# omerbt/Splice

Hardware: AMD Instinct MI355X
Metric: opt_steps_per_sec (higher is better)
Workload: dtype bf16

## Files before the change

include/splice_hip.h:

```cpp
#ifndef SPLICE_HIP_H
#define SPLICE_HIP_H
#include <stddef.h>
#include <stdint.h>

#ifdef __cplusplus
extern "C" {
#endif

typedef uint16_t splice_bf16;
typedef void* splice_stream_t;

#define SPLICE_OK 0
#define SPLICE_ERR_ARG -1
#define SPLICE_ERR_HIP -2
#define SPLICE_ERR_STATE -3
#define SPLICE_ERR_NOMEM -4

int splice_version(void);
int splice_dev_switches(void);
const char* splice_last_error(void);

typedef struct splice_gemm_epilogue {
    const float* bias;
    const float* resid;
// ... 280 lines not shown
int splice_rows_finish(int mode, const float* slabs, int n_slabs, size_t slab_stride, int rows, int N, const float* bias, const float* resid, size_t rs,
                       float* out_f32, size_t os, splice_bf16* out_bf, splice_bf16* pre_bf, const splice_bf16* aux, size_t ps, int pre_lo,
                       splice_stream_t stream);

typedef struct splice_gen_conv_args {
    const float* in;
    const float* w;
    const float* bias;
    float* out;
    size_t in_nstride, in_cstride, out_nstride, out_cstride, w_jstride, w_cstride, p_nstride;
    int N, Cin, Hi, Wi, Cout, Ho, Wo, ks, stride, pad;
    int reflect, act, transposed, accumulate;
    float* ws;
    size_t ws_floats;
    int p_group, defer_reduce;
} splice_gen_conv_args;
#define SPLICE_GEN_CONV_FORM_INTS 5
int splice_gen_conv(const splice_gen_conv_args* args, int* form_out, splice_stream_t stream);
int splice_gen_conv_pair(const splice_gen_conv_args* a, const splice_gen_conv_args* b, int* forms_out, splice_stream_t stream);
int splice_gen_conv_reflect_dgrad(const splice_gen_conv_args* args, float* pad_scratch, size_t scratch_floats, splice_stream_t stream);

typedef struct splice_gen_wgrad_args {
    const float* x;
    const float* dy;
    float* ws;
    size_t ws_floats;
    size_t x_nstride, x_cstride, dy_nstride, dy_cstride;
    int N, Cin, Hi, Wi, Cout, Ho, Wo, ks, stride, pad, reflect;
} splice_gen_wgrad_args;
#define SPLICE_GEN_WGRAD_FORM_INTS 6
size_t splice_gen_conv_wgrad_ws_floats(int N, int Cin, int Cout, int ks, int Ho, int Wo);
int splice_gen_conv_wgrad(const splice_gen_wgrad_args* args, float* dw, int accumulate, int n_img, size_t p_nstride, int* form_out,
                          splice_stream_t stream);
int splice_gen_wgrad_reduce(const float* partials, int n, int chunks, float* dw, int accumulate, int n_img, size_t p_nstride, splice_stream_t stream);

typedef struct splice_gen_bn_args {
    float* y;
    float* out;
    size_t y_nstride, out_nstride;
    int N, C, HW, batch;
    const float* gamma;
    const float* beta;
    float eps, slope;
    size_t p_nstride;
    float* part;
    size_t part_floats;
    float* mean;
    float* rstd;
    const float* up_src;
    float* up_d_src;
    size_t up_src_ns, up_d_src_ns;
    int up_c0, up_h, up_w, up_Ho, up_Wo;
    const float* slabs;
    const float* bias;
    int ksplit;
    const float* da;
    float* dy;
    size_t da_nstride, dy_nstride;
    float* dgamma;
    float* dbeta;
    int accumulate;
    const float* da_slabs;
    int da_ksplit, da_accumulate;
    float* pre_y;
    size_t pre_y_ns;
    const float* pre_slabs;
// ... 31 lines not shown
```

splice_amd/_lib.py:

```python
import ctypes as C
import os

_HERE = os.path.dirname(os.path.abspath(__file__))
LIB_PATH = os.path.join(_HERE, "libsplice_hip.so")

_lib = None


class GemmEpilogue(C.Structure):
    _fields_ = [
        ("bias", C.c_void_p), ("resid", C.c_void_p), ("ldr", C.c_int), ("resid_mod", C.c_int),
        ("out_f32", C.c_void_p), ("ldo", C.c_int),
        ("out_bf", C.c_void_p), ("ldbf", C.c_int),
        ("out_bf_t", C.c_void_p), ("ldt", C.c_int),
        ("out_pre", C.c_void_p), ("ldp", C.c_int), ("pre_row_lo", C.c_int),
        ("aux", C.c_void_p), ("ldaux", C.c_int),
        ("out_f32_cols", C.c_void_p), ("ld_cols", C.c_int), ("col_lo", C.c_int), ("col_hi", C.c_int),
        ("alpha", C.c_float), ("ksplit", C.c_int), ("slab_stride", C.c_longlong),
        ("rd_other", C.c_void_p), ("ld_rd", C.c_int), ("rd_rows", C.c_int), ("rowdot", C.c_void_p),
        ("row_scale", C.c_void_p), ("col_scale", C.c_void_p),
        ("out_f8", C.c_void_p), ("ld8", C.c_int),
        ("out_f8_t", C.c_void_p), ("ldt8", C.c_int),
    ]

# ... 78 lines not shown
    "splice_gemm_nt_bf16": ([_u, _vp, _i, _vp, _i, _i, _i, _i, C.POINTER(GemmEpilogue), _vp], _i),
    "splice_gemm_nt_fp8": ([_u, _vp, _i, _vp, _i, _i, _i, _i, C.POINTER(GemmEpilogue), _vp], _i),
    "splice_quantize_rows_fp8": ([_vp, _i, _vp, _i, _vp, _i, _i, _vp], _i),
    "splice_gemm_splitk_slabs": ([_i, _i], _i),
    "splice_gemm_force_tile": ([_i], _i),
    "splice_attention_variant": ([_i], _i),
    "splice_attention_qfold": ([_i], _i),
    "splice_attention_bwd_variant": ([_i], _i),
    "splice_layernorm_fwd": ([_vp, _vp, _vp, _vp, _vp, _vp, _i, _i, _f, _vp], _i),
    "splice_layernorm_bwd": ([_vp, _vp, _vp, _vp, _vp, _vp, _vp, _vp, _i, _i, _vp], _i),
    "splice_attention_fwd": ([_vp, _vp, _i, _i, _i, _i, _i, _i, _f, _vp, _vp, _vp], _i),
    "splice_attention_fwd_fp8": ([_vp, _vp, _i, _i, _i, _i, _i, _i, _f, _vp, _vp, _vp], _i),
    "splice_attention_bwd": ([_vp, _vp, _i, _i, _i, _i, _i, _i, _f, _vp, _vp, _vp, _vp, _vp, _vp, _vp], _i),
    "splice_attention_probs": ([_vp, _i, _i, _i, _i, _i, _f, _vp, _vp, _vp], _i),
    "splice_augment_structure": ([_vp, _vp, _vp, _i, _i, _i, _i, C.POINTER(C.c_int), C.POINTER(C.c_float), _f, _vp], _i),
    "splice_keys_selfsim_ws_bytes": ([_i, _i], _sz),
    "splice_keys_selfsim_fwd": ([_vp, _i, _i, _i, _f, _vp, _vp, _vp], _i),
    "splice_keys_selfsim_bwd": ([_vp, _vp, _i, _i, _f, _vp, _i, _i, _vp, _vp], _i),
    "splice_mse": ([_vp, _i, _vp, _i, _i, _i, _f, _vp, _vp, _i, _vp], _i),
    "splice_selfsim_loss_pairs_ws_bytes": ([_i, _i, _i], _sz),
    "splice_selfsim_loss_pairs": ([_vp, _vp, _i, _sz, _vp, _i, _sz, _i, _i, _i, _f, _vp, _i, _f, _vp, _sz, _vp, _i, _sz, _vp, _vp], _i),
    "splice_mse_pairs": ([_vp, _i, _sz, _vp, _i, _sz, _i, _i, _f, _f, _vp, _sz, _vp, _i, _sz, _i, _vp, _vp], _i),
    "splice_total_loss_pairs": ([_vp, _sz, _i, _f, _f, _f, _f, _f, _vp, _i, _i, _i, _i, _i, _vp, _i, _i, _vp], _i),
    "splice_attn_cls_fwd": ([_vp, _vp, _i, _i, _i, _i, _i, _i, _f, _vp, _vp, _vp], _i),
    "splice_attn_cls_bwd": ([_vp, _vp, _i, _i, _i, _i, _i, _i, _f, _vp, _vp, _i, _sz, _vp, _vp], _i),
    "splice_ln_rows_fwd": ([_vp, _sz, _vp, _vp, _vp, _sz, _vp, _vp, _sz, _i, _i, _f, _vp, _i, _sz, _vp, _vp, _sz, _vp], _i),
    "splice_ln_rows_bwd": ([_vp, _sz, _vp, _sz, _vp, _vp, _vp, _sz, _vp, _vp, _i, _i, _i, _sz, _vp], _i),
    "splice_rows_finish": ([_i, _vp, _i, _sz, _i, _i, _vp, _vp, _sz, _vp, _sz, _vp, _vp, _vp, _sz, _i, _vp], _i),
    "splice_gen_conv": ([C.POINTER(GenConvArgs), C.POINTER(_i), _vp], _i),
    "splice_gen_conv_pair": ([C.POINTER(GenConvArgs), C.POINTER(GenConvArgs), C.POINTER(_i), _vp], _i),
    "splice_gen_conv_reflect_dgrad": ([C.POINTER(GenConvArgs), _vp, _sz, _vp], _i),
    "splice_gen_conv_wgrad_ws_floats": ([_i, _i, _i, _i, _i, _i], _sz),
    "splice_gen_conv_wgrad": ([C.POINTER(GenWgradArgs), _vp, _i, _i, _sz, C.POINTER(_i), _vp], _i),
    "splice_gen_wgrad_reduce": ([_vp, _i, _i, _vp, _i, _i, _sz, _vp], _i),
    "splice_gen_bn_small_instance": ([_i], _i),
    "splice_gen_bn_form": ([_i, _i, _sz, _i, C.POINTER(_i)], _i),
    "splice_gen_bn_part_floats": ([_i, _i], _sz),
    "splice_gen_bn_fwd": ([C.POINTER(GenBnArgs), _vp], _i),
    "splice_gen_bn_bwd": ([C.POINTER(GenBnArgs), _vp], _i),
    "splice_gen_upsample2x_fwd": ([_vp, _sz, _vp, _sz, _i, _i, _i, _i, _i, _i, _vp], _i),
    "splice_gen_upsample2x_bwd": ([_vp, _sz, _vp, _sz, _i, _i, _i, _i, _i, _i, _vp], _i),
    "splice_gen_sigmoid_bias_part_floats": ([_i, _i], _sz),
    "splice_gen_sigmoid_bwd_bias": ([_vp, _vp, _vp, _i, _i, _i, _vp, _sz, _sz, _i, C.POINTER(_i), _vp], _i),
    "splice_patchify": ([_vp, _vp, _i, _i, _i, _i, _i, _i, _vp], _i),
    "splice_unpatchify": ([_vp, _vp, _i, _i, _i, _i, _i, _i, _vp], _i),
    "splice_cast_f32_bf16": ([_vp, _vp, _sz, _vp], _i),
    "splice_cast_bf16_f32": ([_vp, _vp, _sz, _vp], _i),
    "splice_transpose_f32_bf16": ([_vp, _vp, _i, _i, _i, _vp], _i),
    "splice_resize_bilinear_fwd": ([_vp, _vp, _i, _i, _i, _i, _i, _vp], _i),
    "splice_resize_bilinear_bwd": ([_vp, _vp, _i, _i, _i, _i, _i, _vp], _i),
    "splice_vit_create": ([_i, _i, _i, _i, C.POINTER(_vp)], _i),
    "splice_vit_destroy": ([_vp], None),
    "splice_vit_set_param": ([_vp, C.c_char_p, _vp, C.c_longlong, _vp], _i),
    "splice_vit_params_complete": ([_vp], _i),
    "splice_vit_enable_fp8": ([_vp, _vp], _i),
    "splice_vit_ctx_create": ([_vp, _i, _i, _i, _vp, _i, _vp, C.POINTER(_vp)], _i),
    "splice_vit_ctx_destroy": ([_vp], None),
    "splice_vit_ctx_info": ([_vp, C.POINTER(_i), C.POINTER(_i), C.POINTER(_i)], _i),
    "splice_vit_ctx_set_top_cls_only": ([_vp, _i], _i),
    "splice_vit_ctx_set_fp8": ([_vp, _i], _i),
    "splice_vit_forward": ([_vp, _vp, _i, _vp], _i),
    "splice_vit_forward_ex": ([_vp, _vp, _i, _i, _vp], _i),
    "splice_vit_forward_passes": ([_vp, _vp, _i, _i, _i, _i, _vp], _i),
    "splice_vit_get_tensor": ([_vp, _i, _i, C.POINTER(_vp)], _i),
    "splice_vit_qscale": ([_vp], C.c_float),
    "splice_vit_read_tensor": ([_vp, _i, _i, _vp, _sz, _vp], _i),
# ... 103 lines not shown
```

splice_amd/csrc/capi.hip:

```cpp
#include <stdarg.h>
#include <stdio.h>

#include "gen_kernels.h"
#include "kernels.h"

static thread_local char g_err[512] = "";

void splice_set_error(const char* fmt, ...) {
    va_list ap;
    va_start(ap, fmt);
    vsnprintf(g_err, sizeof(g_err), fmt, ap);
    va_end(ap);
}

static int finish(int rc, const char* what) {
    if (rc != SPLICE_OK) {
        splice_set_error("%s: invalid argument", what);
        return rc;
    }
    const hipError_t e = hipGetLastError();
    if (e != hipSuccess) {
        splice_set_error("%s: HIP error %d (%s)", what, (int)e, hipGetErrorString(e));
        return SPLICE_ERR_HIP;
    }
// ... 252 lines not shown
    return (size_t)wgrad_chunks(N, Ho, Wo, &ppc, &cpi) * Cout * Cin * ks * ks;
}
int splice_gen_conv_wgrad(const splice_gen_wgrad_args* args, float* dw, int accumulate, int n_img, size_t p_nstride, int* form_out, splice_stream_t stream) {
    const char* who = "splice_gen_conv_wgrad";
    if (!gen_wgrad_args_ok(args) || !dw || !args->ws) return finish(SPLICE_ERR_ARG, who);
    const size_t n = (size_t)args->Cout * args->Cin * args->ks * args->ks;
    if (n > 0x7fffffffULL || args->ws_floats < splice_gen_conv_wgrad_ws_floats(args->N, args->Cin, args->Cout, args->ks, args->Ho, args->Wo))
        return finish(SPLICE_ERR_ARG, who);
    if (p_nstride ? (n_img != args->N || p_nstride < n) : n_img != 1) return finish(SPLICE_ERR_ARG, who);
    WgradArgs a = {};
    a.x = args->x; a.dy = args->dy; a.ws = args->ws;
    a.x_nstride = args->x_nstride; a.x_cstride = args->x_cstride; a.dy_nstride = args->dy_nstride; a.dy_cstride = args->dy_cstride;
    a.N = args->N; a.Cin = args->Cin; a.Hi = args->Hi; a.Wi = args->Wi; a.Cout = args->Cout; a.Ho = args->Ho; a.Wo = args->Wo;
    a.ks = args->ks; a.stride = args->stride; a.pad = args->pad; a.reflect = args->reflect;
    WgradBatchPair pair = {};
    int chunks = 0;
    int rc = conv_wgrad_add(&pair, a, &chunks);
    if (rc != SPLICE_OK) return finish(rc, who);
    WgradReduceAll r = {};
    r.count = 1; r.n[0] = (int)n; r.chunks[0] = chunks; r.ws_off[0] = 0; r.dw_off[0] = 0;
    if (form_out) {
        const WgradBatch& b = pair.tile.count ? pair.tile : pair.big.count ? pair.big : pair.small;
        form_out[0] = pair.tile.count ? 2 : pair.big.count ? 1 : 0;
        form_out[1] = b.d[0].variant;
        form_out[2] = b.d[0].pix_per_chunk;
        form_out[3] = chunks;
        form_out[4] = !((reinterpret_cast<size_t>(args->ws) | reinterpret_cast<size_t>(dw)) & 15) && p_nstride % 4 == 0 && n % 4 == 0;
        form_out[5] = b.total_wgs;
    }
    rc = conv_wgrad_batched_launch(pair, ST(stream));
    if (rc != SPLICE_OK) return finish(rc, who);
    return finish(wgrad_reduce_all_launch(r, args->ws, dw, accumulate, ST(stream), n_img, p_nstride), who);
}

int splice_gen_wgrad_reduce(const float* partials, int n, int chunks, float* dw, int accumulate, int n_img, size_t p_nstride, splice_stream_t stream) {
    const char* who = "splice_gen_wgrad_reduce";
    if (!partials || !dw || n < 1 || chunks < 0 || n_img < 1 || n_img > 65535 || (long long)n * (chunks > 0 ? chunks : 1) > 0x7fffffffLL) return finish(SPLICE_ERR_ARG, who);
    if (p_nstride ? (chunks % n_img || p_nstride < (size_t)n) : n_img != 1) return finish(SPLICE_ERR_ARG, who);
    WgradReduceAll r = {};
    r.count = 1; r.n[0] = n; r.chunks[0] = chunks; r.ws_off[0] = 0; r.dw_off[0] = 0;
    return finish(wgrad_reduce_all_launch(r, partials, dw, accumulate, ST(stream), n_img, p_nstride), who);
}

int splice_gen_bn_small_instance(int mask) { return finish(bn_small_force_instance(mask), "splice_gen_bn_small_instance"); }
int splice_gen_bn_form(int HW, int N, size_t p_nstride, int batch, int* out) {
    if (HW < 1 || N < 1 || batch < 0 || !out) return finish(SPLICE_ERR_ARG, "splice_gen_bn_form");
    const BnForm f = bn_form(HW, N, p_nstride, batch);
    out[0] = (int)f.kind; out[1] = f.hosts_pre; out[2] = f.fwd_takes_slabs; out[3] = f.bwd_takes_slabs;
    out[4] = f.fwd_fuses_upsample; out[5] = f.bwd_fuses_upsample; out[6] = f.sign_from_y;
    return SPLICE_OK;
}
size_t splice_gen_bn_part_floats(int N, int C) { return N < 1 || C < 1 ? 0 : (size_t)bn_part_floats(N, C); }
static bool gen_bn_fill(const splice_gen_bn_args* g, bool bwd, BnArgs* a, BnUpsample* up, BnPre* pre, BnSlabs* sl) {
    if (!g || !g->y || !g->out || !g->gamma || !g->mean || !g->rstd) return false;
    if (g->N < 1 || g->C < 1 || g->HW < 1 || g->N > 65535 || g->C > 65535 || g->batch < 0 || g->batch > 8) return false;
    if (g->batch && (g->N % g->batch || (g->N != g->batch && !g->p_nstride))) return false;
    if (g->N > 1 && (g->y_nstride < (size_t)g->C * g->HW || g->out_nstride < (size_t)g->C * g->HW)) return false;
    const BnForm f = bn_form(g->HW, g->N, g->p_nstride, g->batch);
    const bool two_stage = f.kind == BnForm::TWO_STAGE || f.kind == BnForm::TWO_STAGE_VEC;
    if (two_stage && (!g->part || g->part_floats < (size_t)bn_part_floats(g->N, g->C))) return false;
    if (!bwd && !g->beta) return false;
    if (bwd && ((f.sign_from_y && !g->beta) || !g->da || !g->dy || !g->dgamma || !g->dbeta)) return false;
    if (bwd && g->N > 1 && (g->da_nstride < (size_t)g->C * g->HW || g->dy_nstride < (size_t)g->C * g->HW)) return false;
    a->y = g->y; a->y_nstride = g->y_nstride; a->out = g->out; a->out_nstride = g->out_nstride;
    a->N = g->N; a->C = g->C; a->HW = g->HW; a->gamma = g->gamma; a->beta = g->beta; a->eps = g->eps; a->slope = g->slope;
    a->p_nstride = g->p_nstride; a->batch = g->batch; a->part = g->part; a->mean = g->mean; a->rstd = g->rstd;
// ... 95 lines not shown
```

splice_amd/csrc/gen_wgrad.hip:

```cpp
#include "gen_device.h"
#include <cstdlib>

constexpr int WG_PC = 64;
constexpr int WG_LD = WG_PC + 2;
constexpr int WG_XS_FLOATS = 3 * 16 * WG_LD;
constexpr int WG_DS_FLOATS = 8 * 16 * WG_LD;
template <int KS, int NI, bool ROWS = false>
__device__ __forceinline__ void conv_wgrad_body(const WgradArgs& a, int chunk, int ktile_in, float* Xs, float* Ds) {
    constexpr int T = ROWS ? KS : KS * KS;
    constexpr int CK = (ROWS || KS == 3) ? 4 : 16;
    constexpr int KT = CK * T;
    const int ktile = ROWS ? ktile_in / KS : ktile_in;
    const int krow = ROWS ? ktile_in % KS : 0;
    constexpr int NJ = (KT + 15) / 16;
    constexpr int PC = WG_PC;
    constexpr int LD = WG_LD;
    constexpr int NQ = (NI * NJ + 3) / 4;
    constexpr int NA = KT / 4;
    constexpr int ND = NI * 16 * PC / 256;
    const int tid = threadIdx.x, lane = tid & 63, wave = tid >> 6;
    const int c0 = ktile * CK;
    const int HWo = a.Ho * a.Wo;
    const int chunks_per_img = a.chunks_per_img;
    const int img = chunk / chunks_per_img, ch_in_img = chunk % chunks_per_img;
    const float* x = a.x + (size_t)img * a.x_nstride + (size_t)c0 * a.x_cstride;
    const float* dy = a.dy + (size_t)img * a.dy_nstride;
    f32x4 acc[NQ];
#pragma unroll
    for (int q = 0; q < NQ; ++q) acc[q] = f32x4{0.f, 0.f, 0.f, 0.f};
    for (int e = tid; e < (NJ * 16 - KT) * LD; e += 256) Xs[KT * LD + e] = 0.f;
    const int pl = tid & 63;
    const int p_begin = ch_in_img * a.pix_per_chunk;
    const int p_end = min(p_begin + a.pix_per_chunk, HWo);
    const int wave_g = (KS == 3 && NI == 8) ? __builtin_amdgcn_readfirstlane(wave) : wave;
    int g_coff[NA], g_dy[NA], g_dx[NA];
    unsigned g_cok = 0;
#pragma unroll
    for (int i = 0; i < NA; ++i) {
        const int k = wave_g + 4 * i;
        const int cl = k / T, tap = k % T;
        g_coff[i] = (int)(cl * a.x_cstride);
        g_dy[i] = (ROWS ? krow : tap / KS) - a.pad;
        g_dx[i] = (ROWS ? tap : tap % KS) - a.pad;
        if (c0 + cl < a.Cin) g_cok |= 1u << i;
    }
    float xv[NA], dv[ND];
    const __amdgpu_buffer_rsrc_t rx = __builtin_amdgcn_make_buffer_rsrc(const_cast<float*>(x), 0, 0x7FFFFFFF, 0x00020000);
    const __amdgpu_buffer_rsrc_t rdy = __builtin_amdgcn_make_buffer_rsrc(const_cast<float*>(dy), 0, 0x7FFFFFFF, 0x00020000);
    int d_vo[ND];
#pragma unroll
    for (int t = 0; t < ND; ++t) {
        const int e = tid + 256 * t;
        const int n = e / PC, q = e % PC;
        d_vo[t] = n < a.Cout ? (int)((n * a.dy_cstride + q) * 4) : (int)0x80000000;
    }
    auto fetch = [&](int pb) {
        const int p = pb + pl;
        const bool pvalid = p < p_end;
        const int oy = pvalid ? p / a.Wo : 0, ox = pvalid ? p % a.Wo : 0;
        const int by = oy * a.stride, bx = ox * a.stride;
#pragma unroll
        for (int i = 0; i < NA; ++i) {
            int sy = by + g_dy[i], sx = bx + g_dx[i];
            if (a.reflect) {
                sy = sy < 0 ? -sy : (sy >= a.Hi ? 2 * (a.Hi - 1) - sy : sy);
                sx = sx < 0 ? -sx : (sx >= a.Wi ? 2 * (a.Wi - 1) - sx : sx);
            }
            const bool ok = pvalid && ((g_cok >> i) & 1u) && (unsigned)sy < (unsigned)a.Hi && (unsigned)sx < (unsigned)a.Wi;
            const int vo = ok ? (g_coff[i] + sy * a.Wi + sx) * 4 : (int)0x80000000;
            xv[i] = __builtin_bit_cast(float, __builtin_amdgcn_raw_buffer_load_b32(rx, vo, 0, 0));
        }
        if (pb + PC <= p_end) {
            const int so = __builtin_amdgcn_readfirstlane(pb * 4);
#pragma unroll
            for (int t = 0; t < ND; ++t) dv[t] = __builtin_bit_cast(float, __builtin_amdgcn_raw_buffer_load_b32(rdy, d_vo[t], so, 0));
        } else {
#pragma unroll
            for (int t = 0; t < ND; ++t) {
                const int e = tid + 256 * t;
                const int n = e / PC, q = e % PC;
                const int pp = pb + q;
                dv[t] = (n < a.Cout && pp < p_end) ? dy[(size_t)n * a.dy_cstride + pp] : 0.f;
            }
        }
    };
    fetch(p_begin);
    constexpr int WB = 4, NB = PC / 4 / WB;
    [[maybe_unused]] int lds_rd = (lane & 15) * LD + (lane >> 4);
    for (int pb = p_begin; pb < p_end; pb += PC) {
        if constexpr (NI < 4) asm volatile("" : "+v"(lds_rd));
        __syncthreads();
#pragma unroll
        for (int i = 0; i < NA; ++i) Xs[(wave + 4 * i) * LD + pl] = xv[i];
#pragma unroll
        for (int t = 0; t < ND; ++t) {
            const int e = tid + 256 * t;
            Ds[(e / PC) * LD + (e % PC)] = dv[t];
        }
        __syncthreads();
        if (pb + PC < p_end) fetch(pb + PC);
#pragma unroll
        for (int q = 0; q < NQ; ++q) {
            const int pair = wave + 4 * q;
            if (pair < NI * NJ) {
                const int fi = pair / NJ, fj = pair % NJ;
                if constexpr (NI >= 4) {
#pragma unroll
                    for (int s4 = 0; s4 < PC / 4; ++s4) {
                        const float av = Ds[(fi * 16 + (lane & 15)) * LD + s4 * 4 + (lane >> 4)];
                        const float bv = Xs[(fj * 16 + (lane & 15)) * LD + s4 * 4 + (lane >> 4)];
                        acc[q] = mfma4(av, bv, acc[q]);
                    }
                } else {
                    const int d_rd = lds_rd + fi * 16 * LD, x_rd = lds_rd + fj * 16 * LD;
                    float af[2][WB], bf[2][WB];
#pragma unroll
                    for (int t = 0; t < WB; ++t) { af[0][t] = Ds[d_rd + t * 4]; bf[0][t] = Xs[x_rd + t * 4]; }
#pragma unroll
                    for (int b = 0; b < NB; ++b) {
                        if (b + 1 < NB) {
#pragma unroll
                            for (int t = 0; t < WB; ++t) { af[(b + 1) & 1][t] = Ds[d_rd + ((b + 1) * WB + t) * 4]; bf[(b + 1) & 1][t] = Xs[x_rd + ((b + 1) * WB + t) * 4]; }
                        }
                        __builtin_amdgcn_sched_barrier(0);
#pragma unroll
                        for (int t = 0; t < WB; ++t) acc[q] = mfma4(af[b & 1][t], bf[b & 1][t], acc[q]);
                        __builtin_amdgcn_sched_barrier(0);
                    }
                }
            }
        }
    }
    constexpr int TT = KS * KS;
    float* ws = a.ws + (size_t)chunk * a.Cout * a.Cin * TT;
#pragma unroll
    for (int q = 0; q < NQ; ++q) {
        const int pair = wave + 4 * q;
        if (pair < NI * NJ) {
            const int fi = pair / NJ, fj = pair % NJ;
            const int k = fj * 16 + (lane & 15);
            const int cl = k / T, tap = k % T;
            if (k < KT && c0 + cl < a.Cin) {
#pragma unroll
                for (int r = 0; r < 4; ++r) {
                    const int n = fi * 16 + (lane >> 4) * 4 + r;
                    if (n < a.Cout) ws[((size_t)n * a.Cin + c0 + cl) * TT + (ROWS ? krow * KS + tap : tap)] = acc[q][r];
                }
            }
        }
    }
}

__device__ __forceinline__ void wgrad_loaded(float& x) { asm volatile("" : "+v"(x) : : "memory"); }
template <class Load>
__device__ __forceinline__ float wgrad_chunk_sum(int chunks, Load&& ld) {
    float s0 = 0.f, s1 = 0.f, s2 = 0.f, s3 = 0.f;
    int c = 0;
#pragma unroll 1
    for (; c + 31 < chunks; c += 32) {
        float v[32];
#pragma unroll
        for (int u = 0; u < 32; ++u) v[u] = ld(c + u);
#pragma unroll
        for (int u = 0; u < 32; ++u) wgrad_loaded(v[u]);
#pragma unroll
        for (int u = 0; u < 32; u += 4) { s0 += v[u]; s1 += v[u + 1]; s2 += v[u + 2]; s3 += v[u + 3]; }
    }
    for (; c + 15 < chunks; c += 16) {
        float v[16];
#pragma unroll
        for (int u = 0; u < 16; ++u) v[u] = ld(c + u);
#pragma unroll
        for (int u = 0; u < 16; u += 4) { s0 += v[u]; s1 += v[u + 1]; s2 += v[u + 2]; s3 += v[u + 3]; }
    }
    for (; c + 3 < chunks; c += 4) {
        s0 += ld(c);
        s1 += ld(c + 1);
        s2 += ld(c + 2);
        s3 += ld(c + 3);
    }
    for (; c < chunks; ++c) s0 += ld(c);
    return (s0 + s1) + (s2 + s3);
}
// ... 61 lines not shown
            a1.x += v1.x; a1.y += v1.y; a1.z += v1.z; a1.w += v1.w;
            a2.x += v2.x; a2.y += v2.y; a2.z += v2.z; a2.w += v2.w;
            a3.x += v3.x; a3.y += v3.y; a3.z += v3.z; a3.w += v3.w;
        }
        for (; c < chunks; ++c) {
            const float4 v0 = *reinterpret_cast<const float4*>(p + (size_t)c * n);
            a0.x += v0.x; a0.y += v0.y; a0.z += v0.z; a0.w += v0.w;
        }
        s.x = (a0.x + a1.x) + (a2.x + a3.x); s.y = (a0.y + a1.y) + (a2.y + a3.y);
        s.z = (a0.z + a1.z) + (a2.z + a3.z); s.w = (a0.w + a1.w) + (a2.w + a3.w);
        float4* q4 = reinterpret_cast<float4*>(q);
        if (accumulate) { const float4 o = *q4; s.x = o.x + s.x; s.y = o.y + s.y; s.z = o.z + s.z; s.w = o.w + s.w; }
        *q4 = s;
        return;
    }
    const float s = wgrad_chunk_sum(chunks, [&](int c) { return p[(size_t)c * n]; });
    *q = accumulate ? *q + s : s;
}

int wgrad_chunks(int N, int Ho, int Wo, int* pix_per_chunk, int* chunks_per_img) {
    const int HWo = Ho * Wo;
    int ppc = 512;
    if (HWo <= 1024) ppc = 256;
    if (HWo <= 256) ppc = 64;
    if (HWo > 128 * 512) ppc = (cdiv(HWo, 128) + 63) / 64 * 64;
    *pix_per_chunk = ppc;
    *chunks_per_img = cdiv(HWo, ppc);
    return N * *chunks_per_img;
}

template <bool BIG>
__global__ __launch_bounds__(256, 2) void conv_wgrad_batched_kernel(WgradBatch b) {
    __shared__ float Xs[WG_XS_FLOATS];
    __shared__ float Ds[(BIG ? 8 : 2) * 16 * WG_LD];
    int l = 0;
#pragma unroll 1
    while (l + 1 < b.count && blockIdx.x >= b.d[l + 1].wg_begin) ++l;
    const WgradDesc& d = b.d[l];
    WgradArgs a;
    a.x = d.x; a.dy = d.dy; a.ws = d.ws;
    a.x_nstride = d.x_nstride; a.x_cstride = d.x_cstride; a.dy_nstride = d.dy_nstride; a.dy_cstride = d.dy_cstride;
    a.N = 0; a.Cin = d.Cin; a.Hi = d.Hi; a.Wi = d.Wi; a.Cout = d.Cout; a.Ho = d.Ho; a.Wo = d.Wo;
    a.ks = d.ks; a.stride = d.stride; a.pad = d.pad; a.pix_per_chunk = d.pix_per_chunk; a.chunks_per_img = d.chunks_per_img;
    a.reflect = (int)d.reflect;
    const int local = blockIdx.x - d.wg_begin;
    const int chunk = local % d.chunks, ktile = local / d.chunks;
    if (BIG) {
        switch (d.variant) {
            case 2: conv_wgrad_body<1, 4>(a, chunk, ktile, Xs, Ds); break;
            case 3: conv_wgrad_body<1, 8>(a, chunk, ktile, Xs, Ds); break;
            case 6: conv_wgrad_body<3, 4>(a, chunk, ktile, Xs, Ds); break;
            case 7: conv_wgrad_body<3, 8>(a, chunk, ktile, Xs, Ds); break;
            case 10: conv_wgrad_body<5, 4, true>(a, chunk, ktile, Xs, Ds); break;
            case 11: conv_wgrad_body<5, 8, true>(a, chunk, ktile, Xs, Ds); break;
            case 14: conv_wgrad_body<7, 4, true>(a, chunk, ktile, Xs, Ds); break;
            default: conv_wgrad_body<7, 8, true>(a, chunk, ktile, Xs, Ds); break;
        }
    } else {
        switch (d.variant) {
            case 0: conv_wgrad_body<1, 1>(a, chunk, ktile, Xs, Ds); break;
            case 1: conv_wgrad_body<1, 2>(a, chunk, ktile, Xs, Ds); break;
            case 4: conv_wgrad_body<3, 1>(a, chunk, ktile, Xs, Ds); break;
            case 5: conv_wgrad_body<3, 2>(a, chunk, ktile, Xs, Ds); break;
            case 8: conv_wgrad_body<5, 1, true>(a, chunk, ktile, Xs, Ds); break;
            case 9: conv_wgrad_body<5, 2, true>(a, chunk, ktile, Xs, Ds); break;
            case 12: conv_wgrad_body<7, 1, true>(a, chunk, ktile, Xs, Ds); break;
            default: conv_wgrad_body<7, 2, true>(a, chunk, ktile, Xs, Ds); break;
// ... 151 lines not shown
    else conv_wgrad_tile_body<2>(d, chunk, ktile, nb, Ps);
}
static bool wgrad_tile_ok(const WgradArgs& a) {
    static const int on = getenv("SPLICE_WGRAD_TILE") ? atoi(getenv("SPLICE_WGRAD_TILE")) : 1;
    constexpr int min_px = 40000;
    return on && a.ks == 3 && a.stride == 1 && a.Wo >= 64 && (long long)a.Ho * a.Wo > min_px && a.Hi == a.Ho && a.Wi == a.Wo && a.pad == 1 &&
           (size_t)a.Cin * a.x_cstride <= 0x1fffffffULL && (size_t)a.Cout * a.dy_cstride <= 0x1fffffffULL;
}

int conv_wgrad_add(WgradBatchPair* pair, WgradArgs a, int* chunks_out) {
    const bool tile = wgrad_tile_ok(a);
    WgradBatch* b = tile ? &pair->tile : a.Cout > 32 ? &pair->big : &pair->small;
    if (a.Cout > 128 || (a.ks != 1 && a.ks != 3 && a.ks != 5 && a.ks != 7) || b->count >= WGRAD_BATCH_MAX) return SPLICE_ERR_ARG;
    if ((size_t)a.Cin * a.x_cstride > 0x7fffffffULL || a.x_nstride > 0xffffffffULL || a.dy_nstride > 0xffffffffULL) return SPLICE_ERR_ARG;
    if (a.Hi > 65535 || a.Wi > 65535 || a.Cin > 65535) return SPLICE_ERR_ARG;
    const int chunks = wgrad_chunks(a.N, a.Ho, a.Wo, &a.pix_per_chunk, &a.chunks_per_img);
    const int CK = tile ? WT_CK : a.ks == 1 ? 16 : 4;
    const int ktiles = cdiv(a.Cin, CK) * (a.ks >= 5 ? a.ks : 1) * (tile ? cdiv(a.Cout, 32) : 1);
    const int ni = cdiv(a.Cout, 16);
    WgradDesc& d = b->d[b->count++];
    d.x = a.x; d.dy = a.dy; d.ws = a.ws;
    d.x_nstride = (uint32_t)a.x_nstride; d.x_cstride = (uint32_t)a.x_cstride; d.dy_nstride = (uint32_t)a.dy_nstride; d.dy_cstride = (uint32_t)a.dy_cstride;
    d.Cin = (uint16_t)a.Cin; d.Cout = (uint16_t)a.Cout; d.Hi = (uint16_t)a.Hi; d.Wi = (uint16_t)a.Wi; d.Ho = (uint16_t)a.Ho; d.Wo = (uint16_t)a.Wo;
    d.ks = (uint8_t)a.ks; d.stride = (uint8_t)a.stride; d.pad = (uint8_t)a.pad;
    d.variant = (uint8_t)((a.ks == 3 ? 4 : a.ks == 5 ? 8 : a.ks == 7 ? 12 : 0) + (ni <= 1 ? 0 : ni <= 2 ? 1 : ni <= 4 ? 2 : 3));
    if (tile) d.variant = (uint8_t)(ni < 2 ? 1 : 2);
    d.reflect = (uint32_t)(a.reflect ? 1 : 0);
    d.pix_per_chunk = (uint16_t)a.pix_per_chunk; d.chunks_per_img = (uint16_t)a.chunks_per_img;
    d.wg_begin = (uint32_t)b->total_wgs; d.chunks = (uint32_t)chunks;
    b->total_wgs += chunks * ktiles;
    if (chunks_out) *chunks_out = chunks;
    return SPLICE_OK;
}
int conv_wgrad_batched_launch(const WgradBatchPair& p, hipStream_t s) {
    if (p.big.count > 0) SPLICE_LAUNCH(conv_wgrad_batched_kernel<true>, dim3((unsigned)p.big.total_wgs), dim3(256), 0, s, p.big);
    if (p.small.count > 0) SPLICE_LAUNCH(conv_wgrad_batched_kernel<false>, dim3((unsigned)p.small.total_wgs), dim3(256), 0, s, p.small);
    if (p.tile.count > 0) SPLICE_LAUNCH(conv_wgrad_tile_kernel, dim3((unsigned)p.tile.total_wgs), dim3(256), 0, s, p.tile);
    return SPLICE_OK;
}

int wgrad_reduce_all_launch(const WgradReduceAll& d0, const float* ws, float* grads, int accumulate, hipStream_t s, int n_img, size_t p_nstride) {
    if (d0.count < 1 || d0.count > WGRAD_MAX_LAYERS) return SPLICE_ERR_ARG;
    WgradReduceAll d = d0;
    static const int vec_on = getenv("SPLICE_WGRAD_REDUCE_VEC") ? atoi(getenv("SPLICE_WGRAD_REDUCE_VEC")) : 1;
    const bool base_ok = vec_on && !((reinterpret_cast<size_t>(ws) | reinterpret_cast<size_t>(grads)) & 15) && p_nstride % 4 == 0;
    d.prefix[0] = 0;
    for (int i = 0; i < d.count; ++i) {
        const bool v = base_ok && d.n[i] % 4 == 0 && d.ws_off[i] % 4 == 0 && d.dw_off[i] % 4 == 0;
        d.vec[i] = v ? 1 : 0;
        d.prefix[i + 1] = d.prefix[i] + (v ? d.n[i] / 4 : d.n[i]);
    }
    d.total = d.prefix[d.count];
    SPLICE_LAUNCH(wgrad_reduce_all_kernel, dim3((unsigned)((d.total + 255) / 256), p_nstride ? n_img : 1), dim3(256), 0, s, d, ws, grads, accumulate,
                       n_img, p_nstride);
    return SPLICE_OK;
}
```

Before: 271.0.

## Restructure wgrad MFMA tiling with per-wave fragment blocks, vector dy loads, heavy-first scheduling

The conv weight-gradient body now gives each wave a fixed block of output fragments (FI x FJ) instead of striding over fragment pairs, so A/B values read from LDS are reused across several MFMAs. dy is fetched with 128-bit buffer loads and stored to LDS as float4, with padding widened to LD=68 and an XOR swizzle to limit bank conflicts. Batched launches reorder layer descriptors so the heaviest layers get their workgroups first, reducing tail imbalance. A new batch C API entry point that adds several layers to one launch and reduces each is also exposed. This adds register pressure from larger accumulator arrays and more complex swizzle logic.

```diff
diff --git a/include/splice_hip.h b/include/splice_hip.h
--- a/include/splice_hip.h
+++ b/include/splice_hip.h
@@ -336,6 +336,7 @@
 size_t splice_gen_conv_wgrad_ws_floats(int N, int Cin, int Cout, int ks, int Ho, int Wo);
 int splice_gen_conv_wgrad(const splice_gen_wgrad_args* args, float* dw, int accumulate, int n_img, size_t p_nstride, int* form_out,
                           splice_stream_t stream);
+int splice_gen_conv_wgrad_batch(const splice_gen_wgrad_args* layers, int count, float* const* dw, splice_stream_t stream);
 int splice_gen_wgrad_reduce(const float* partials, int n, int chunks, float* dw, int accumulate, int n_img, size_t p_nstride, splice_stream_t stream);
 
 typedef struct splice_gen_bn_args {
diff --git a/splice_amd/_lib.py b/splice_amd/_lib.py
--- a/splice_amd/_lib.py
+++ b/splice_amd/_lib.py
@@ -134,6 +134,7 @@
     "splice_gen_conv_reflect_dgrad": ([C.POINTER(GenConvArgs), _vp, _sz, _vp], _i),
     "splice_gen_conv_wgrad_ws_floats": ([_i, _i, _i, _i, _i, _i], _sz),
     "splice_gen_conv_wgrad": ([C.POINTER(GenWgradArgs), _vp, _i, _i, _sz, C.POINTER(_i), _vp], _i),
+    "splice_gen_conv_wgrad_batch": ([C.POINTER(GenWgradArgs), _i, C.POINTER(_vp), _vp], _i),
     "splice_gen_wgrad_reduce": ([_vp, _i, _i, _vp, _i, _i, _sz, _vp], _i),
     "splice_gen_bn_small_instance": ([_i], _i),
     "splice_gen_bn_form": ([_i, _i, _sz, _i, C.POINTER(_i)], _i),
diff --git a/splice_amd/csrc/capi.hip b/splice_amd/csrc/capi.hip
--- a/splice_amd/csrc/capi.hip
+++ b/splice_amd/csrc/capi.hip
@@ -308,6 +308,32 @@
     if (rc != SPLICE_OK) return finish(rc, who);
     return finish(wgrad_reduce_all_launch(r, args->ws, dw, accumulate, ST(stream), n_img, p_nstride), who);
 }
+int splice_gen_conv_wgrad_batch(const splice_gen_wgrad_args* layers, int count, float* const* dw, splice_stream_t stream) {
+    const char* who = "splice_gen_conv_wgrad_batch";
+    if (!layers || !dw || count < 1 || count > WGRAD_BATCH_MAX) return finish(SPLICE_ERR_ARG, who);
+    WgradBatchPair pair = {};
+    int chunks[WGRAD_BATCH_MAX];
+    for (int i = 0; i < count; ++i) {
+        const splice_gen_wgrad_args* g = layers + i;
+        if (!gen_wgrad_args_ok(g) || !dw[i] || !g->ws) return finish(SPLICE_ERR_ARG, who);
+        const size_t n = (size_t)g->Cout * g->Cin * g->ks * g->ks;
+        if (n > 0x7fffffffULL || g->ws_floats < splice_gen_conv_wgrad_ws_floats(g->N, g->Cin, g->Cout, g->ks, g->Ho, g->Wo)) return finish(SPLICE_ERR_ARG, who);
+        WgradArgs a = {};
+        a.x = g->x; a.dy = g->dy; a.ws = g->ws;
+        a.x_nstride = g->x_nstride; a.x_cstride = g->x_cstride; a.dy_nstride = g->dy_nstride; a.dy_cstride = g->dy_cstride;
+        a.N = g->N; a.Cin = g->Cin; a.Hi = g->Hi; a.Wi = g->Wi; a.Cout = g->Cout; a.Ho = g->Ho; a.Wo = g->Wo;
+        a.ks = g->ks; a.stride = g->stride; a.pad = g->pad; a.reflect = g->reflect;
+        const int rc = conv_wgrad_add(&pair, a, &chunks[i]);
+        if (rc != SPLICE_OK) return finish(rc, who);
+    }
+    int rc = conv_wgrad_batched_launch(pair, ST(stream));
+    for (int i = 0; i < count && rc == SPLICE_OK; ++i) {
+        WgradReduceAll r = {};
+        r.count = 1; r.n[0] = layers[i].Cout * layers[i].Cin * layers[i].ks * layers[i].ks; r.chunks[0] = chunks[i]; r.ws_off[0] = 0; r.dw_off[0] = 0;
+        rc = wgrad_reduce_all_launch(r, layers[i].ws, dw[i], 0, ST(stream), 1, 0);
+    }
+    return finish(rc, who);
+}
 
 int splice_gen_wgrad_reduce(const float* partials, int n, int chunks, float* dw, int accumulate, int n_img, size_t p_nstride, splice_stream_t stream) {
     const char* who = "splice_gen_wgrad_reduce";
diff --git a/splice_amd/csrc/gen_wgrad.hip b/splice_amd/csrc/gen_wgrad.hip
--- a/splice_amd/csrc/gen_wgrad.hip
+++ b/splice_amd/csrc/gen_wgrad.hip
@@ -1,8 +1,10 @@
 #include "gen_device.h"
+#include <algorithm>
 #include <cstdlib>
+#include <type_traits>
 
 constexpr int WG_PC = 64;
-constexpr int WG_LD = WG_PC + 2;
+constexpr int WG_LD = WG_PC + 4;
 constexpr int WG_XS_FLOATS = 3 * 16 * WG_LD;
 constexpr int WG_DS_FLOATS = 8 * 16 * WG_LD;
 template <int KS, int NI, bool ROWS = false>
@@ -15,9 +17,11 @@
     constexpr int NJ = (KT + 15) / 16;
     constexpr int PC = WG_PC;
     constexpr int LD = WG_LD;
-    constexpr int NQ = (NI * NJ + 3) / 4;
+    constexpr int FI = NI >= 8 ? 2 : 1;
+    constexpr int FJ = NI >= 4 ? NJ : NI == 2 ? (NJ + 1) / 2 : 1;
+    static_assert(NI >= 4 || FJ <= 2, "a ragged share is 1 of 2 k fragments");
     constexpr int NA = KT / 4;
-    constexpr int ND = NI * 16 * PC / 256;
+    constexpr int ND = NI * 16 * PC / 256 / 4;
     const int tid = threadIdx.x, lane = tid & 63, wave = tid >> 6;
     const int c0 = ktile * CK;
     const int HWo = a.Ho * a.Wo;
@@ -25,9 +29,15 @@
     const int img = chunk / chunks_per_img, ch_in_img = chunk % chunks_per_img;
     const float* x = a.x + (size_t)img * a.x_nstride + (size_t)c0 * a.x_cstride;
     const float* dy = a.dy + (size_t)img * a.dy_nstride;
-    f32x4 acc[NQ];
-#pragma unroll
-    for (int q = 0; q < NQ; ++q) acc[q] = f32x4{0.f, 0.f, 0.f, 0.f};
+    const int wave_u = __builtin_amdgcn_readfirstlane(wave);
+    const int fi0 = NI >= 4 ? wave_u * FI : NI == 2 ? (wave_u & 1) : 0;
+    const int fj0 = NI >= 4 ? 0 : NI == 2 ? (wave_u >> 1) * FJ : wave_u;
+    const int njw = min(FJ, NJ - fj0);
+    f32x4 acc[FI][FJ];
+#pragma unroll
+    for (int i = 0; i < FI; ++i)
+#pragma unroll
+        for (int j = 0; j < FJ; ++j) acc[i][j] = f32x4{0.f, 0.f, 0.f, 0.f};
     for (int e = tid; e < (NJ * 16 - KT) * LD; e += 256) Xs[KT * LD + e] = 0.f;
     const int pl = tid & 63;
     const int p_begin = ch_in_img * a.pix_per_chunk;
@@ -44,15 +54,16 @@
         g_dx[i] = (ROWS ? tap : tap % KS) - a.pad;
         if (c0 + cl < a.Cin) g_cok |= 1u << i;
     }
-    float xv[NA], dv[ND];
+    float xv[NA];
+    f32x4 dv[ND];
     const __amdgpu_buffer_rsrc_t rx = __builtin_amdgcn_make_buffer_rsrc(const_cast<float*>(x), 0, 0x7FFFFFFF, 0x00020000);
     const __amdgpu_buffer_rsrc_t rdy = __builtin_amdgcn_make_buffer_rsrc(const_cast<float*>(dy), 0, 0x7FFFFFFF, 0x00020000);
+    const int d_run = (tid & 15) * 4, d_row = tid >> 4;
     int d_vo[ND];
 #pragma unroll
     for (int t = 0; t < ND; ++t) {
-        const int e = tid + 256 * t;
-        const int n = e / PC, q = e % PC;
-        d_vo[t] = n < a.Cout ? (int)((n * a.dy_cstride + q) * 4) : (int)0x80000000;
+        const int n = d_row + 16 * t;
+        d_vo[t] = n < a.Cout ? (int)((n * a.dy_cstride + d_run) * 4) : (int)0x80000000;
     }
     auto fetch = [&](int pb) {
         const int p = pb + pl;
@@ -70,85 +81,101 @@
             const int vo = ok ? (g_coff[i] + sy * a.Wi + sx) * 4 : (int)0x80000000;
             xv[i] = __builtin_bit_cast(float, __builtin_amdgcn_raw_buffer_load_b32(rx, vo, 0, 0));
         }
+        const int so = __builtin_amdgcn_readfirstlane(pb * 4);
         if (pb + PC <= p_end) {
-            const int so = __builtin_amdgcn_readfirstlane(pb * 4);
-#pragma unroll
-            for (int t = 0; t < ND; ++t) dv[t] = __builtin_bit_cast(float, __builtin_amdgcn_raw_buffer_load_b32(rdy, d_vo[t], so, 0));
+#pragma unroll
+            for (int t = 0; t < ND; ++t) dv[t] = __builtin_bit_cast(f32x4, __builtin_amdgcn_raw_buffer_load_b128(rdy, d_vo[t], so, 0));
         } else {
 #pragma unroll
-            for (int t = 0; t < ND; ++t) {
-                const int e = tid + 256 * t;
-                const int n = e / PC, q = e % PC;
-                const int pp = pb + q;
-                dv[t] = (n < a.Cout && pp < p_end) ? dy[(size_t)n * a.dy_cstride + pp] : 0.f;
-            }
+            for (int t = 0; t < ND; ++t)
+#pragma unroll
+                for (int k = 0; k < 4; ++k) {
+                    const bool ok = d_vo[t] >= 0 && pb + d_run + k < p_end;
+                    dv[t][k] = __builtin_bit_cast(float, __builtin_amdgcn_raw_buffer_load_b32(rdy, ok ? d_vo[t] + 4 * k : (int)0x80000000, so, 0));
+                }
         }
     };
     fetch(p_begin);
     constexpr int WB = 4, NB = PC / 4 / WB;
-    [[maybe_unused]] int lds_rd = (lane & 15) * LD + (lane >> 4);
+    int lds_rd = (lane & 15) * LD + ((lane >> 4) ^ ((lane >> 2) & 2));
+    auto mma_fill = [&](auto njc) __attribute__((always_inline)) {
+        constexpr int NJW = decltype(njc)::value;
+        const int d_rd = lds_rd + fi0 * 16 * LD, x_rd = lds_rd + fj0 * 16 * LD;
+        if constexpr (NI >= 4) {
+#pragma unroll
+            for (int s4 = 0; s4 < PC / 4; ++s4) {
+                float av[FI], bv[NJW];
+#pragma unroll
+                for (int i = 0; i < FI; ++i) av[i] = Ds[d_rd + i * 16 * LD + s4 * 4];
+#pragma unroll
+                for (int j = 0; j < NJW; ++j) bv[j] = Xs[x_rd + j * 16 * LD + s4 * 4];
+#pragma unroll
+                for (int i = 0; i < FI; ++i)
+#pragma unroll
+                    for (int j = 0; j < NJW; ++j) acc[i][j] = mfma4(av[i], bv[j], acc[i][j]);
+            }
+        } else {
+            float af[2][WB][FI], bf[2][WB][NJW];
+            auto rd = [&](int b) __attribute__((always_inline)) {
+#pragma unroll
+                for (int t = 0; t < WB; ++t) {
+#pragma unroll
+                    for (int i = 0; i < FI; ++i) af[b & 1][t][i] = Ds[d_rd + i * 16 * LD + (b * WB + t) * 4];
+#pragma unroll
+                    for (int j = 0; j < NJW; ++j) bf[b & 1][t][j] = Xs[x_rd + j * 16 * LD + (b * WB + t) * 4];
+                }
+            };
+            rd(0);
+#pragma unroll
+            for (int b = 0; b < NB; ++b) {
+                if (b + 1 < NB) rd(b + 1);
+                __builtin_amdgcn_sched_barrier(0);
+#pragma unroll
+                for (int t = 0; t < WB; ++t)
+#pragma unroll
+                    for (int i = 0; i < FI; ++i)
+#pragma unroll
+                        for (int j = 0; j < NJW; ++j) acc[i][j] = mfma4(af[b & 1][t][i], bf[b & 1][t][j], acc[i][j]);
+                __builtin_amdgcn_sched_barrier(0);
+            }
+        }
+    };
     for (int pb = p_begin; pb < p_end; pb += PC) {
-        if constexpr (NI < 4) asm volatile("" : "+v"(lds_rd));
+        asm volatile("" : "+v"(lds_rd));
         __syncthreads();
 #pragma unroll
-        for (int i = 0; i < NA; ++i) Xs[(wave + 4 * i) * LD + pl] = xv[i];
+        for (int i = 0; i < NA; ++i) Xs[(wave + 4 * i) * LD + (pl ^ (i & 2))] = xv[i];
 #pragma unroll
         for (int t = 0; t < ND; ++t) {
-            const int e = tid + 256 * t;
-            Ds[(e / PC) * LD + (e % PC)] = dv[t];
+            const f32x4 v = dv[t];
+            *reinterpret_cast<f32x4*>(&Ds[(d_row + 16 * t) * LD + d_run]) = (wave_u & 2) ? f32x4{v[2], v[3], v[0], v[1]} : v;
         }
         __syncthreads();
         if (pb + PC < p_end) fetch(pb + PC);
-#pragma unroll
-        for (int q = 0; q < NQ; ++q) {
-            const int pair = wave + 4 * q;
-            if (pair < NI * NJ) {
-                const int fi = pair / NJ, fj = pair % NJ;
-                if constexpr (NI >= 4) {
-#pragma unroll
-                    for (int s4 = 0; s4 < PC / 4; ++s4) {
-                        const float av = Ds[(fi * 16 + (lane & 15)) * LD + s4 * 4 + (lane >> 4)];
-                        const float bv = Xs[(fj * 16 + (lane & 15)) * LD + s4 * 4 + (lane >> 4)];
-                        acc[q] = mfma4(av, bv, acc[q]);
-                    }
-                } else {
-                    const int d_rd = lds_rd + fi * 16 * LD, x_rd = lds_rd + fj * 16 * LD;
-                    float af[2][WB], bf[2][WB];
-#pragma unroll
-                    for (int t = 0; t < WB; ++t) { af[0][t] = Ds[d_rd + t * 4]; bf[0][t] = Xs[x_rd + t * 4]; }
-#pragma unroll
-                    for (int b = 0; b < NB; ++b) {
-                        if (b + 1 < NB) {
-#pragma unroll
-                            for (int t = 0; t < WB; ++t) { af[(b + 1) & 1][t] = Ds[d_rd + ((b + 1) * WB + t) * 4]; bf[(b + 1) & 1][t] = Xs[x_rd + ((b + 1) * WB + t) * 4]; }
-                        }
-                        __builtin_amdgcn_sched_barrier(0);
-#pragma unroll
-                        for (int t = 0; t < WB; ++t) acc[q] = mfma4(af[b & 1][t], bf[b & 1][t], acc[q]);
-                        __builtin_amdgcn_sched_barrier(0);
-                    }
-                }
-            }
+        if (FJ == 1 || njw == FJ) {
+            if (njw > 0) mma_fill(std::integral_constant<int, FJ>{});
+        } else if (njw > 0) {
+            mma_fill(std::integral_constant<int, 1>{});
         }
     }
     constexpr int TT = KS * KS;
     float* ws = a.ws + (size_t)chunk * a.Cout * a.Cin * TT;
 #pragma unroll
-    for (int q = 0; q < NQ; ++q) {
-        const int pair = wave + 4 * q;
-        if (pair < NI * NJ) {
-            const int fi = pair / NJ, fj = pair % NJ;
+    for (int i = 0; i < FI; ++i)
+#pragma unroll
+        for (int j = 0; j < FJ; ++j) {
+            if (j >= njw) continue;
+            const int fi = fi0 + i, fj = fj0 + j;
             const int k = fj * 16 + (lane & 15);
             const int cl = k / T, tap = k % T;
             if (k < KT && c0 + cl < a.Cin) {
 #pragma unroll
                 for (int r = 0; r < 4; ++r) {
                     const int n = fi * 16 + (lane >> 4) * 4 + r;
-                    if (n < a.Cout) ws[((size_t)n * a.Cin + c0 + cl) * TT + (ROWS ? krow * KS + tap : tap)] = acc[q][r];
+                    if (n < a.Cout) ws[((size_t)n * a.Cin + c0 + cl) * TT + (ROWS ? krow * KS + tap : tap)] = acc[i][j][r];
                 }
             }
         }
-    }
 }
 
 __device__ __forceinline__ void wgrad_loaded(float& x) { asm volatile("" : "+v"(x) : : "memory"); }
@@ -276,7 +303,7 @@
 template <bool BIG>
 __global__ __launch_bounds__(256, 2) void conv_wgrad_batched_kernel(WgradBatch b) {
     __shared__ float Xs[WG_XS_FLOATS];
-    __shared__ float Ds[(BIG ? 8 : 2) * 16 * WG_LD];
+    __shared__ __attribute__((aligned(16))) float Ds[(BIG ? 8 : 2) * 16 * WG_LD];
     int l = 0;
 #pragma unroll 1
     while (l + 1 < b.count && blockIdx.x >= b.d[l + 1].wg_begin) ++l;
@@ -494,7 +521,28 @@
     if (chunks_out) *chunks_out = chunks;
     return SPLICE_OK;
 }
-int conv_wgrad_batched_launch(const WgradBatchPair& p, hipStream_t s) {
+static WgradBatch wgrad_heavy_first(const WgradBatch& b0) {
+    WgradBatch b = b0;
+    int idx[WGRAD_BATCH_MAX], wgs[WGRAD_BATCH_MAX], weight[WGRAD_BATCH_MAX];
+    for (int i = 0; i < b0.count; ++i) {
+        const WgradDesc& d = b0.d[i];
+        const int nj[4] = {1, 3, 2, 2};
+        idx[i] = i;
+        wgs[i] = (int)((i + 1 < b0.count ? b0.d[i + 1].wg_begin : (uint32_t)b0.total_wgs) - d.wg_begin);
+        weight[i] = cdiv(std::min<int>(d.pix_per_chunk, d.Ho * d.Wo), WG_PC) * (nj[d.variant >> 2] << (d.variant & 3));
+    }
+    std::stable_sort(idx, idx + b0.count, [&](int x, int y) { return weight[x] > weight[y]; });
+    uint32_t begin = 0;
+    for (int i = 0; i < b0.count; ++i) {
+        b.d[i] = b0.d[idx[i]];
+        b.d[i].wg_begin = begin;
+        begin += (uint32_t)wgs[idx[i]];
+    }
+    return b;
+}
+int conv_wgrad_batched_launch(const WgradBatchPair& p0, hipStream_t s) {
+    WgradBatchPair p;
+    p.big = wgrad_heavy_first(p0.big); p.small = wgrad_heavy_first(p0.small); p.tile = p0.tile;
     if (p.big.count > 0) SPLICE_LAUNCH(conv_wgrad_batched_kernel<true>, dim3((unsigned)p.big.total_wgs), dim3(256), 0, s, p.big);
     if (p.small.count > 0) SPLICE_LAUNCH(conv_wgrad_batched_kernel<false>, dim3((unsigned)p.small.total_wgs), dim3(256), 0, s, p.small);
     if (p.tile.count > 0) SPLICE_LAUNCH(conv_wgrad_tile_kernel, dim3((unsigned)p.tile.total_wgs), dim3(256), 0, s, p.tile);
```

Measured after the change: 272.6 (median of 6 runs). About the same (+0.6%).
